# PFLeget/treegp

Hardware: AMD Instinct MI355X
Metric: GP solve+predict throughput, 2-D AnisotropicRBF N=65536 (higher is better)
Workload: dtype f64

## Files before the change

include/tgp.h:

```cpp
#ifndef TGP_H
#define TGP_H

#include <stdint.h>

#ifdef __cplusplus
extern "C" {
#endif

typedef struct tgp_ctx tgp_ctx;
typedef struct tgp_factor tgp_factor;

enum {
    TGP_RBF = 0,
    TGP_ARBF = 1,
    TGP_VK = 2,
    TGP_AVK = 3
};

typedef struct {
    int32_t kind;
    int32_t _pad;
    double amp;
    double a, b, c;
    double ell;
// ... 76 lines not shown
                 int k, double *out);

#define TGP_STAT_MEAN 0
#define TGP_STAT_MEDIAN 1
#define TGP_STAT_WEIGHTED 2
int tgp_binned_stat_2d(tgp_ctx *ctx, const double *u, const double *v, const double *val, const double *err,
                       int64_t n, const double *u_edges, int nu_edges, const double *v_edges, int nv_edges,
                       int stat, double *average, double *wrms, double *count);

int tgp_dev_alloc(tgp_ctx *ctx, int64_t bytes, void **d_out);
int tgp_dev_free(tgp_ctx *ctx, void *d_ptr);
int tgp_h2d(tgp_ctx *ctx, void *d_dst, const void *src, int64_t bytes);
int tgp_d2h(tgp_ctx *ctx, void *dst, const void *d_src, int64_t bytes);
int tgp_sync(tgp_ctx *ctx);
void *tgp_stream(tgp_ctx *ctx);
int tgp_mem_info(tgp_ctx *ctx, int64_t *free_bytes, int64_t *total_bytes);

int tgp_d_gp_solve(tgp_ctx *ctx, const tgp_kernel *k, const double *d_X, int64_t n,
                   const double *d_y, const double *d_yerr, double *d_alpha, double *logdet,
                   double *ydota, tgp_factor **keep);
int tgp_d_gp_predict(tgp_ctx *ctx, const tgp_kernel *k, const double *d_X, int64_t n,
                     const double *d_alpha, const double *d_Xs, int64_t m, double *d_ys);
int tgp_d_gp_solve_dense(tgp_ctx *ctx, const double *d_K, int64_t n, const double *d_y,
                         const double *d_yerr, double *d_alpha, double *logdet, double *ydota,
                         tgp_factor **keep);

int64_t tgp_panel_off(int64_t p, int64_t Np);
int64_t tgp_panel_elems(int64_t Np);
int64_t tgp_padded_n(int64_t n);

int tgp_d_kbuild_lower(tgp_ctx *ctx, const tgp_kernel *k, const double *d_X, int64_t n,
                       const double *d_yerr, double *d_A);
int tgp_d_potrf(tgp_ctx *ctx, double *d_A, int64_t Np, double *d_W);
int tgp_d_potrs(tgp_ctx *ctx, const double *d_A, const double *d_W, int64_t Np, double *d_b);
int tgp_d_potrs_multi(tgp_ctx *ctx, const double *d_A, const double *d_W, int64_t Np, double *d_B, int nrhs);
int tgp_d_unpack_lower(tgp_ctx *ctx, const double *d_A, int64_t Np, int64_t n, double *out);
int tgp_factor_device(tgp_ctx *ctx, const tgp_factor *f, const double **d_A, const double **d_W, int64_t *Np);
int tgp_set_stream(tgp_ctx *ctx, void *hip_stream);
int tgp_reset_stream(tgp_ctx *ctx);
int tgp_set_side_stream(tgp_ctx *ctx, void *hip_stream);
int64_t tgp_dist_panel_rows(int64_t p, int64_t Np, int G, int g);
int64_t tgp_dist_panel_off(int64_t p, int64_t Np, int G, int g);
int64_t tgp_dist_local_elems(int64_t Np, int G, int g);
int tgp_dd_kbuild(tgp_ctx *ctx, const tgp_kernel *k, const double *d_X, int64_t n, const double *d_yerr,
                  double *d_Aloc, const int64_t *d_loff, int G, int g);
int tgp_dd_factor_diag(tgp_ctx *ctx, double *d_Aloc, const int64_t *h_loff, int64_t Np, int kpanel, int G, int g,
                       double *d_W, double *d_bcast);
int tgp_dd_trsm(tgp_ctx *ctx, double *d_Aloc, const int64_t *h_loff, int64_t Np, int kpanel, int G, int g,
                double *d_W, const double *d_bcast);
int tgp_dd_update(tgp_ctx *ctx, double *d_Aloc, const int64_t *d_loff, int64_t Np, int kpanel, int G, int g,
                  const double *d_gathered, int cmax, int col_lo, int col_hi);
int tgp_dd_update2(tgp_ctx *ctx, double *d_Aloc, const int64_t *d_loff, int64_t Np, int kpanel, int G, int g,
                   const double *d_gathered0, int cmax0, const double *d_gathered1, int cmax1, int col_lo,
                   int col_hi);
int tgp_dd_update_group(tgp_ctx *ctx, double *d_Aloc, const int64_t *d_loff, int64_t Np, int kpanel, int G, int g,
                        int nseg, const double *const *d_gathered, const int *cmax, int col_lo, int col_hi);
int tgp_dd_strip_left(tgp_ctx *ctx, double *d_Aloc, const int64_t *h_loff, const int64_t *d_loff, int64_t Np, int kgroup, int b,
                      int G, int g, const double *d_ext);
int tgp_dd_queue_reset(tgp_ctx *ctx);
int tgp_dd_set_exclusive(tgp_ctx *ctx, int on);
int tgp_dd_update_group_queued(tgp_ctx *ctx, double *d_Aloc, const int64_t *d_loff, int64_t Np, int kpanel, int G, int g,
                               int nseg, const double *const *d_gathered, const int *cmax, int col_lo, int col_hi, int nres);
int tgp_dd_update_group_fused(tgp_ctx *ctx, double *d_Aloc, const int64_t *d_loff, int64_t Np, int kpanel, int G, int g, int nseg,
                              const double *const *d_gathered, const int *cmax, int head_cols, int nres);
int tgp_dd_wait_head(tgp_ctx *ctx, tgp_ctx *waiter);
int tgp_dd_tail_assemble(tgp_ctx *ctx, const double *d_gathered, int64_t stride, int64_t Np, int k0, int G, double *d_tail);
int tgp_dd_tail_scatter(tgp_ctx *ctx, const double *d_tail, int64_t Np, int k0, int G, int g, double *d_Aloc, const int64_t *d_loff);
int tgp_handoff_mode(tgp_ctx *ctx);
int tgp_dd_keep_panel(tgp_ctx *ctx, double *d_Afull, int64_t Np, int kpanel, int G, const double *d_bcast,
                      const double *d_gathered, int cmax);
int tgp_dd_fwd_diag(tgp_ctx *ctx, const double *d_Aloc, const int64_t *h_loff, int kb, const double *d_W, double *d_yk);
int tgp_dd_fwd_update(tgp_ctx *ctx, const double *d_Aloc, const int64_t *h_loff, int64_t Np, int kb, int G, int g,
                      const double *d_zk, double *d_yloc);
int tgp_dd_bwd_partial(tgp_ctx *ctx, const double *d_Aloc, const int64_t *h_loff, int64_t Np, int kb, int G, int g,
                       const double *d_aloc, double *d_s);
int tgp_dd_bwd_diag(tgp_ctx *ctx, const double *d_Aloc, const int64_t *h_loff, int kb, const double *d_W, double *d_ak,
                    const double *d_s );
int tgp_dd_logdet_local(tgp_ctx *ctx, const double *d_Aloc, const int64_t *d_loff, int64_t Np, int64_t n, int G, int g,
                        double *d_out);
int tgp_dd_info(tgp_ctx *ctx, int reset);

int tgp_debug_syrk_loop(tgp_ctx *ctx, double *d_A, int64_t Np, int reps, double *ms_per_launch,
                        double *flops_per_launch);
int tgp_debug_tilemap(int64_t T, int32_t *ti, int32_t *tj, int64_t cap);

#ifdef __cplusplus
}
#endif
#endif
```

treegp_amd/_lib.py:

```python
import ctypes as C
import os
import threading

import numpy as np

_HERE = os.path.dirname(os.path.abspath(__file__))
LIB_PATH = os.environ.get("TGP_LIB_PATH") or os.path.join(_HERE, "csrc", "libtgp.so")

TGP_RBF, TGP_ARBF, TGP_VK, TGP_AVK = 0, 1, 2, 3
NTIMINGS = 12


class TgpKernel(C.Structure):
    _fields_ = [("kind", C.c_int32), ("_pad", C.c_int32), ("amp", C.c_double), ("a", C.c_double),
                ("b", C.c_double), ("c", C.c_double), ("ell", C.c_double)]


_dp = C.POINTER(C.c_double)
_vp = C.c_void_p
_i64 = C.c_int64

SIGNATURES = {
    "tgp_init": (C.c_int, [C.POINTER(C.c_int), C.c_int, C.POINTER(_vp)]),
    "tgp_destroy": (None, [_vp]),
    "tgp_release_caches": (C.c_int, [_vp]),
    "tgp_last_error": (C.c_char_p, [_vp]),
    "tgp_version": (C.c_char_p, []),
    "tgp_device_count": (C.c_int, []),
    "tgp_last_timings": (C.c_int, [_vp, _dp, C.c_int]),
    "tgp_set_profiling": (C.c_int, [_vp, C.c_int]),
    "tgp_set_lookahead": (C.c_int, [_vp, C.c_int]),
    "tgp_kernel_matrix": (C.c_int, [_vp, C.POINTER(TgpKernel), _vp, _i64, _vp, _i64, _vp]),
    "tgp_gp_solve": (C.c_int, [_vp, C.POINTER(TgpKernel), _vp, _i64, _vp, _vp, _vp, _dp, _dp, C.POINTER(_vp)]),
    "tgp_factor_free": (None, [_vp, _vp]),
    "tgp_factor_release": (None, [_vp, _vp]),
    "tgp_factor_borrow": (C.c_int, [_vp, _vp, _vp, _i64, C.POINTER(_vp)]),
    "tgp_gp_predict": (C.c_int, [_vp, C.POINTER(TgpKernel), _vp, _i64, _vp, _vp, _i64, _vp]),
    "tgp_gp_predict_cov": (C.c_int, [_vp, _vp, C.POINTER(TgpKernel), _vp, _i64, _vp, _i64, _vp]),
    "tgp_kk_twod": (C.c_int, [_vp, _vp, _vp, _vp, _vp, _i64, C.c_double, C.c_double, C.c_int, _vp, _vp, _vp]),
    "tgp_kk_log": (C.c_int, [_vp, _vp, _vp, _vp, _vp, _i64, C.c_double, C.c_double, C.c_int, _vp, _vp, _vp, _vp, _vp]),
    "tgp_kk_partial": (C.c_int, [_vp, C.c_int, _vp, _vp, _vp, _vp, _i64, C.c_double, C.c_double, C.c_int, C.c_int, C.c_int, _vp]),
    "tgp_kk_twod_bootstrap": (C.c_int, [_vp, _vp, _vp, _vp, _vp, _i64, _vp, _i64, C.c_double, C.c_double, C.c_int, _vp]),
    "tgp_vcorr": (C.c_int, [_vp, _vp, _vp, _vp, _vp, _i64, _vp, C.c_int, _vp]),
    "tgp_knn_mean": (C.c_int, [_vp, _vp, _vp, _i64, _vp, _i64, C.c_int, _vp]),
    "tgp_binned_stat_2d": (C.c_int, [_vp, _vp, _vp, _vp, _vp, _i64, _vp, C.c_int, _vp, C.c_int, C.c_int, _vp, _vp, _vp]),
    "tgp_dev_alloc": (C.c_int, [_vp, _i64, C.POINTER(_vp)]),
    "tgp_dev_free": (C.c_int, [_vp, _vp]),
    "tgp_h2d": (C.c_int, [_vp, _vp, _vp, _i64]),
    "tgp_d2h": (C.c_int, [_vp, _vp, _vp, _i64]),
    "tgp_sync": (C.c_int, [_vp]),
    "tgp_stream": (_vp, [_vp]),
    "tgp_mem_info": (C.c_int, [_vp, C.POINTER(_i64), C.POINTER(_i64)]),
    "tgp_d_gp_solve": (C.c_int, [_vp, C.POINTER(TgpKernel), _vp, _i64, _vp, _vp, _vp, _dp, _dp, C.POINTER(_vp)]),
    "tgp_d_gp_predict": (C.c_int, [_vp, C.POINTER(TgpKernel), _vp, _i64, _vp, _vp, _i64, _vp]),
    "tgp_panel_off": (_i64, [_i64, _i64]),
    "tgp_panel_elems": (_i64, [_i64]),
    "tgp_padded_n": (_i64, [_i64]),
    "tgp_d_kbuild_lower": (C.c_int, [_vp, C.POINTER(TgpKernel), _vp, _i64, _vp, _vp]),
    "tgp_d_potrf": (C.c_int, [_vp, _vp, _i64, _vp]),
    "tgp_d_potrs": (C.c_int, [_vp, _vp, _vp, _i64, _vp]),
    "tgp_d_potrs_multi": (C.c_int, [_vp, _vp, _vp, _i64, _vp, C.c_int]),
    "tgp_gp_solve_dense": (C.c_int, [_vp, _vp, _i64, _vp, _vp, _vp, _dp, _dp, C.POINTER(_vp)]),
    "tgp_d_gp_solve_dense": (C.c_int, [_vp, _vp, _i64, _vp, _vp, _vp, _dp, _dp, C.POINTER(_vp)]),
    "tgp_factor_solve": (C.c_int, [_vp, _vp, _vp, C.c_int, _vp]),
    "tgp_factor_lmul": (C.c_int, [_vp, _vp, _vp, C.c_int, _vp]),
    "tgp_factor_inv_diag": (C.c_int, [_vp, _vp, _vp]),
    "tgp_gp_solve_batch": (C.c_int, [_vp, C.c_int, _vp, _vp, _i64, _vp, _vp, _vp, _vp, _vp, _vp, _vp]),
    "tgp_gp_posterior_batch": (C.c_int, [_vp, C.c_int, _vp, _vp, _i64, _vp, _vp, _vp, _vp, _i64, _vp, C.c_int, _vp, _vp, _vp, _vp, _vp]),
    "tgp_gp_predict_cov_dense": (C.c_int, [_vp, _vp, _vp, _vp, _i64, _vp]),
    "tgp_gp_predict_var": (C.c_int, [_vp, _vp, C.POINTER(TgpKernel), _vp, _i64, _vp, _i64, _vp]),
    "tgp_gp_predict_var_dense": (C.c_int, [_vp, _vp, _vp, _vp, _i64, _vp]),
    "tgp_gp_loglik_grad": (C.c_int, [_vp, _vp, C.POINTER(TgpKernel), _vp, _i64, _vp, _vp]),
    "tgp_d_gp_solve_grad": (C.c_int, [_vp, C.POINTER(TgpKernel), _vp, _i64, _vp, _vp, _dp, _dp, _vp]),
    "tgp_d_unpack_lower": (C.c_int, [_vp, _vp, _i64, _i64, _vp]),
    "tgp_factor_device": (C.c_int, [_vp, _vp, C.POINTER(_vp), C.POINTER(_vp), C.POINTER(_i64)]),
    "tgp_debug_syrk_loop": (C.c_int, [_vp, _vp, _i64, C.c_int, _dp, _dp]),
    "tgp_debug_tilemap": (C.c_int, [_i64, _vp, _vp, _i64]),
    "tgp_set_stream": (C.c_int, [_vp, _vp]),
    "tgp_reset_stream": (C.c_int, [_vp]),
    "tgp_set_side_stream": (C.c_int, [_vp, _vp]),
    "tgp_dist_panel_rows": (_i64, [_i64, _i64, C.c_int, C.c_int]),
    "tgp_dist_panel_off": (_i64, [_i64, _i64, C.c_int, C.c_int]),
    "tgp_dist_local_elems": (_i64, [_i64, C.c_int, C.c_int]),
    "tgp_dd_kbuild": (C.c_int, [_vp, C.POINTER(TgpKernel), _vp, _i64, _vp, _vp, _vp, C.c_int, C.c_int]),
    "tgp_dd_factor_diag": (C.c_int, [_vp, _vp, _vp, _i64, C.c_int, C.c_int, C.c_int, _vp, _vp]),
    "tgp_dd_trsm": (C.c_int, [_vp, _vp, _vp, _i64, C.c_int, C.c_int, C.c_int, _vp, _vp]),
    "tgp_dd_update": (C.c_int, [_vp, _vp, _vp, _i64, C.c_int, C.c_int, C.c_int, _vp, C.c_int, C.c_int, C.c_int]),
    "tgp_dd_update2": (C.c_int, [_vp, _vp, _vp, _i64, C.c_int, C.c_int, C.c_int, _vp, C.c_int, _vp, C.c_int, C.c_int, C.c_int]),
    "tgp_dd_update_group": (C.c_int, [_vp, _vp, _vp, _i64, C.c_int, C.c_int, C.c_int, C.c_int, _vp, _vp, C.c_int, C.c_int]),
    "tgp_dd_strip_left": (C.c_int, [_vp, _vp, _vp, _vp, _i64, C.c_int, C.c_int, C.c_int, C.c_int, _vp]),
    "tgp_dd_update_group_queued": (C.c_int, [_vp, _vp, _vp, _i64, C.c_int, C.c_int, C.c_int, C.c_int, _vp, _vp, C.c_int, C.c_int, C.c_int]),
    "tgp_dd_update_group_fused": (C.c_int, [_vp, _vp, _vp, _i64, C.c_int, C.c_int, C.c_int, C.c_int, _vp, _vp, C.c_int, C.c_int]),
    "tgp_dd_wait_head": (C.c_int, [_vp, _vp]),
    "tgp_handoff_mode": (C.c_int, [_vp]),
    "tgp_dd_tail_assemble": (C.c_int, [_vp, _vp, _i64, _i64, C.c_int, C.c_int, _vp]),
    "tgp_dd_tail_scatter": (C.c_int, [_vp, _vp, _i64, C.c_int, C.c_int, C.c_int, _vp, _vp]),
    "tgp_dd_queue_reset": (C.c_int, [_vp]),
    "tgp_dd_set_exclusive": (C.c_int, [_vp, C.c_int]),
    "tgp_dd_keep_panel": (C.c_int, [_vp, _vp, _i64, C.c_int, C.c_int, _vp, _vp, C.c_int]),
    "tgp_dd_fwd_diag": (C.c_int, [_vp, _vp, _vp, C.c_int, _vp, _vp]),
    "tgp_dd_fwd_update": (C.c_int, [_vp, _vp, _vp, _i64, C.c_int, C.c_int, C.c_int, _vp, _vp]),
    "tgp_dd_bwd_partial": (C.c_int, [_vp, _vp, _vp, _i64, C.c_int, C.c_int, C.c_int, _vp, _vp]),
    "tgp_dd_bwd_diag": (C.c_int, [_vp, _vp, _vp, C.c_int, _vp, _vp, _vp]),
    "tgp_dd_logdet_local": (C.c_int, [_vp, _vp, _vp, _i64, _i64, C.c_int, C.c_int, _vp]),
    "tgp_dd_info": (C.c_int, [_vp, C.c_int]),
}

_lib = None
_ctx = {}
_lock = threading.Lock()


def _share_hip_runtime_with_torch():
    import sys
    if "torch" in sys.modules or os.environ.get("TGP_SYSTEM_HIP") == "1":
        return
    try:
        import importlib.util
        spec = importlib.util.find_spec("torch")
        if spec is None or not spec.origin:
            return
        cand = os.path.join(os.path.dirname(spec.origin), "lib", "libamdhip64.so")
        if os.path.exists(cand):
            C.CDLL(cand, mode=C.RTLD_GLOBAL)
            if os.environ.get("TGP_VERBOSE"):
                print("treegp_amd: using torch's HIP runtime %s (one HIP runtime per process)" % cand, file=sys.stderr)
    except Exception:
        pass


def load_library():
    global _lib
    if _lib is None:
        if not os.path.exists(LIB_PATH):
            raise RuntimeError("libtgp.so not built (%s); run `python -c 'import __graft_entry__ as g; g.build()'` "
                               "or `make -C treegp_amd/csrc`" % LIB_PATH)
        _share_hip_runtime_with_torch()
        if os.environ.get("TGP_SET_HW_QUEUES", "1") != "0":
            os.environ.setdefault("GPU_MAX_HW_QUEUES", "8")
        lib = C.CDLL(LIB_PATH)
        for name, (res, args) in SIGNATURES.items():
            fn = getattr(lib, name)
            fn.restype = res
            fn.argtypes = args
        _lib = lib
    return _lib


class TgpError(RuntimeError):
    pass


_thread = threading.local()


def set_thread_ctx(ctx):
    _thread.ctx = ctx


def release_process_caches(device):
# ... 85 lines not shown
```

treegp_amd/csrc/chol.hip:

```cpp
#include "tgp_internal.h"

#include "gemm_tile.h"
#include "potrf128.h"

#ifdef TGP_POTRF_STAMPS
__device__ unsigned long long tgp_gemm_stamps[1024 * 4];
__device__ int tgp_gemm_stamp_grid = 43;
__device__ unsigned long long tgp_queue_stamps[1024 * 4];
__device__ int tgp_queue_stamp_T = 40;
__device__ unsigned long long tgp_mid_stamps[25 * 8];
__device__ int tgp_mid_stamp_base = 5120;
#define TGP_MID_STAMP(i)                                                                                   \
    do {                                                                                                   \
        if (threadIdx.x == 0 && base == tgp_mid_stamp_base && blockIdx.x < 25) tgp_mid_stamps[blockIdx.x * 8 + (i)] = __builtin_amdgcn_s_memrealtime(); \
    } while (0)
#else
#define TGP_MID_STAMP(i) ((void)0)
#endif

namespace {
template <int MODE, int LDB>
__global__ __launch_bounds__(256, 2) void gemm_col_kernel(const double *A, const double *B, double *C) {
    const int64_t t = blockIdx.x;
    TGP_CHAIN_PRIO();
// ... 504 lines not shown
            return hipFuncSetAttribute((const void *)panel_mid_kernel<true>, hipFuncAttributeMaxDynamicSharedMemorySize, (int)pad) == hipSuccess &&
                   hipFuncSetAttribute((const void *)panel_mid_kernel<false>, hipFuncAttributeMaxDynamicSharedMemorySize, (int)pad) == hipSuccess;
        }();
        const unsigned dyn = (exclusive && pad_ok) ? pad : 0u;
        if (17 + 8 * r2 <= cu_budget) panel_mid_kernel<true><<<25 + 8 * r2, 256, dyn, st>>>(Pk, W0, W1, d_info, base, mid_sync);
        else panel_mid_kernel<false><<<25 + r2, 256, dyn, st>>>(Pk, W0, W1, d_info, base, mid_sync);
    } else if (cu_budget > 0) {
        double *R2 = Pk + (int64_t)TGP_PW * TGP_PW;
        const bool small = 17 + 8 * r2 <= cu_budget;
        gemm_col_small_kernel<0, TGP_TB><<<8, 256, 0, st>>>(R1, W0, R1);
        if (r2 > 0) {
            if (small) gemm_col_small_kernel<0, TGP_TB><<<r2 * 8, 256, 0, st>>>(R2, W0, R2);
            else gemm_col_kernel<0, TGP_TB><<<r2, 256, 0, st>>>(R2, W0, R2);
        }
        gemm_col_small_kernel<1, TGP_PW><<<8, 256, 0, st>>>(R1, R1, R1 + TGP_TB);
        if (r2 > 0) {
            if (small) gemm_col_small_kernel<1, TGP_PW><<<r2 * 8, 256, 0, st>>>(R2, R1, R2 + TGP_TB);
            else gemm_col_kernel<1, TGP_PW><<<r2, 256, 0, st>>>(R2, R1, R2 + TGP_TB);
        }
        run_potrf128(st, R1 + TGP_TB, TGP_PW, W1, d_info, base + TGP_TB, exclusive, solo);
    } else {
        if (r1 <= small_rows) {
            gemm_col_small_kernel<0, TGP_TB><<<r1 * 8, 256, 0, st>>>(R1, W0, R1);
            gemm_col_small_kernel<1, TGP_PW><<<r1 * 8, 256, 0, st>>>(R1, R1, R1 + TGP_TB);
        } else {
            gemm_col_kernel<0, TGP_TB><<<r1, 256, 0, st>>>(R1, W0, R1);
            gemm_col_kernel<1, TGP_PW><<<r1, 256, 0, st>>>(R1, R1, R1 + TGP_TB);
        }
        run_potrf128(st, R1 + TGP_TB, TGP_PW, W1, d_info, base + TGP_TB, exclusive, solo);
    }
    if (r2 > 0) {
        double *R2 = Pk + (int64_t)TGP_PW * TGP_PW + TGP_TB;
        if (r2 <= small_rows) gemm_col_small_kernel<0, TGP_TB><<<r2 * 8, 256, 0, st>>>(R2, W1, R2);
        else gemm_col_kernel<0, TGP_TB><<<r2, 256, 0, st>>>(R2, W1, R2);
    }
}

inline int small_t() {
    static const int v = [] { const char *e = getenv("TGP_SMALL_T"); return e ? atoi(e) : 8; }();
    return v;
}

template <int NSEG>
void launch_syrk(hipStream_t st, double *d_A, int64_t Np, int ob, int T, int strip, const double *P0, const double *P1) {
    if (T <= 0) return;
    static const int strip_small_t = [] { const char *e = getenv("TGP_STRIP_SMALL_T"); return e ? atoi(e) : 16; }();
    if (T <= small_t() || (strip > 0 && T <= strip_small_t)) {
        const int cols = strip == 0 ? T : (strip < T ? strip : T);
        syrk_small_kernel<NSEG><<<dim3((unsigned)(T * 8), (unsigned)cols), 256, 0, st>>>(d_A, Np, ob, T, P0, P1);
        return;
    }
    static const int strip64_t = [] { const char *e = getenv("TGP_STRIP64_T"); return e ? atoi(e) : 128; }();
    static const int strip32_t = [] { const char *e = getenv("TGP_STRIP32_T"); return e ? atoi(e) : 64; }();
    if (strip > 0 && T <= strip32_t) {
        syrk_strip32_kernel<NSEG><<<(unsigned)((int64_t)4 * T * strip), 256, 0, st>>>(d_A, Np, ob, T, strip, P0, P1);
        return;
    }
    if (strip > 0 && T <= strip64_t) {
        syrk_strip64_kernel<NSEG><<<(unsigned)((int64_t)2 * T * strip), 256, 0, st>>>(d_A, Np, ob, T, strip, P0, P1);
        return;
    }
    const unsigned gs = strip == 0 ? (unsigned)tilemap_grid(T) : (unsigned)((int64_t)T * strip);
    syrk_dtv_kernel<NSEG><<<gs, 256, 0, st>>>(d_A, Np, ob, T, strip, P0, P1);
}

int queued_nres(int T) {
    static const int queue_res = [] { const char *e = getenv("TGP_QUEUE_RES"); return e ? atoi(e) : 0; }();
    if (queue_res > 0) return queue_res > TGP_QUEUE_MAXRES ? TGP_QUEUE_MAXRES : queue_res;
    static const int t1 = [] { const char *e = getenv("TGP_QUEUE_T1"); return e ? atoi(e) : 42; }();
    static const int t2 = [] { const char *e = getenv("TGP_QUEUE_T2"); return e ? atoi(e) : 26; }();
    return T >= t1 ? 1 : (T >= t2 ? 2 : 3);
}
void launch_syrk2_queued(tgp_ctx *ctx, hipStream_t st, double *d_A, int64_t Np, int ob, int T, const double *P0, const double *P1,
                         int nqueue) {
    const int nres = queued_nres(T);
    static const int half_env = [] { const char *e = getenv("TGP_QUEUE_HALF"); return e ? atoi(e) : -1; }();
    const unsigned slots = (unsigned)(tilemap_grid(T) / 8);
    unsigned nhalf = half_env >= 0 ? (unsigned)half_env : (unsigned)(512 - 64 * nres) / 8u;
    if (nhalf > slots) nhalf = slots;
    static const int steal = [] { const char *e = getenv("TGP_QUEUE_STEAL"); return e ? atoi(e) : 1; }();
    syrk_dtv_queue_kernel<2><<<512 + 8, 256, 0, st>>>(d_A, Np, ob, T, slots + nhalf, slots - nhalf, nres,
                                                     ctx->d_queue + TGP_QUEUE_WORDS * nqueue, P0, P1, steal);
}
}

int launch_potrf(tgp_ctx *ctx, double *d_A, int64_t Np, double *d_W, bool defer_info, int64_t n_data) {
    TGP_ARG(Np > 0 && Np % TGP_PW == 0);
    hipStream_t st = ctx->stream;
    TGP_HIP(hipMemsetAsync(ctx->d_info, 0, sizeof(int), st));
    const int nP = (int)(Np / TGP_PW);
    const bool prof = ctx->profiling != 0;
    if (prof) {
        while ((int)ctx->prof_events.size() < 2 * nP) {
            hipEvent_t e;
            TGP_HIP(hipEventCreate(&e));
            ctx->prof_events.push_back(e);
        }
    }
    static const int mode_env = [] { const char *e = getenv("TGP_CHOL_MODE"); return e ? atoi(e) : -1; }();
    const int mode = mode_env >= 0 ? mode_env : (!ctx->lookahead ? 1 : (Np >= 18432 ? 3 : (Np <= 1280 ? 1 : 2)));
    if (mode >= 2) {
        int rc = tgp_ensure_side_stream(ctx);
        if (rc) return rc;
    }
    double flops = 0.0;
    int nlaunch = 0;
    bool counting = true;
    auto timed = [&](auto &&fn, double fl) -> int {
        if (!counting) {
            fn();
            return 0;
        }
        if (prof) TGP_HIP(hipEventRecord(ctx->prof_events[2 * nlaunch], st));
        fn();
        if (prof) TGP_HIP(hipEventRecord(ctx->prof_events[2 * nlaunch + 1], st));
        flops += fl;
        ++nlaunch;
        return 0;
    };
    auto Wk = [&](int k) { return d_W + (int64_t)(2 * k) * TGP_TB * TGP_TB; };
    auto panel = [&](int k) { return d_A + panel_off(k, Np); };
    static const int queue_t = [] { const char *e = getenv("TGP_QUEUE_T"); return e ? atoi(e) : 64; }();
    int nqueue = 0;
    static const bool mid_env = [] { const char *e = getenv("TGP_PANEL_MID"); return e ? atoi(e) != 0 : true; }();
    const bool mid_on = mid_env && !ctx->mid_off && ctx->mid_allowed;
    if (mid_on) TGP_HIP(hipMemsetAsync(ctx->d_psync, 0, (size_t)(nP < TGP_PSYNC_PANELS ? nP : TGP_PSYNC_PANELS) * PANEL_SYNC_WORDS * sizeof(unsigned), st));
    if (Np / TGP_TB - 8 > small_t())
        TGP_HIP(hipMemsetAsync(ctx->d_queue, 0, TGP_NQUEUE * TGP_QUEUE_WORDS * sizeof(unsigned), st));
    auto psync = [&](int k) { return (mid_on && k < TGP_PSYNC_PANELS) ? ctx->d_psync + PANEL_SYNC_WORDS * k : nullptr; };
    auto run_pairs = [&](int kstart) -> int {
        hipStream_t sd = ctx->side_stream;
        auto factor_pair = [&](hipStream_t s, int k, bool exclusive = false, int cus = 0, bool tell = false) {
            const int64_t mk = Np - (int64_t)TGP_PW * k;
            auto sync = [&](int kk) { return (cus > 0 && mid_on && kk < TGP_PSYNC_PANELS) ? ctx->d_psync + PANEL_SYNC_WORDS * kk : nullptr; };
            factor_panel(s, panel(k), mk, Wk(k), ctx->d_info, k * TGP_PW, exclusive, n_data, sync(k), cus);
            if (tell) (void)tgp_signal(ctx, s, 2, ctx->ev[6]);
            if (k + 1 >= nP) return;
            const int T1 = (int)((mk - TGP_PW) / TGP_TB);
            launch_syrk<1>(s, d_A, Np, k + 1, T1, 2, panel(k) + (int64_t)TGP_PW * TGP_PW, nullptr);
            factor_panel(s, panel(k + 1), mk - TGP_PW, Wk(k + 1), ctx->d_info, (k + 1) * TGP_PW, exclusive, n_data, sync(k + 1), cus);
        };
        factor_pair(st, kstart, false, 256);
        static const int split_t = [] { const char *e = getenv("TGP_U2A_SPLIT_T"); return e ? atoi(e) : 64; }();
        bool early = false;
        for (int k = kstart; k + 2 < nP; k += 2) {
            const int T2 = (int)((Np - (int64_t)TGP_PW * (k + 2)) / TGP_TB);
            const double *P0 = panel(k) + (int64_t)2 * TGP_PW * TGP_PW;
            const double *P1 = panel(k + 1) + (int64_t)TGP_PW * TGP_PW;
            const int T3 = T2 - 4;
            const bool queued = T3 <= queue_t && T3 > small_t() && nqueue < TGP_NQUEUE;
            {
                const double rows = (double)T2 * TGP_TB, w = (T2 < 4 ? T2 : 4) * (double)TGP_TB;
                const double elems = w * (rows - w) + w * (w + 1.0) / 2.0;
                int rc = timed([&] {
                    if (early) launch_syrk<1>(st, d_A, Np, k + 2, T2, 4, P1, nullptr);
                    else launch_syrk<2>(st, d_A, Np, k + 2, T2, 4, P0, P1);
                }, (early ? 1.0 : 2.0) * 2.0 * TGP_PW * elems);
                if (rc) return rc;
            }
            TGP_HIP(tgp_signal(ctx, st, 0, ctx->ev[4]));
            TGP_HIP(tgp_await(ctx, sd, 0, ctx->ev[4]));
            const bool early_next = T3 > 0 && T3 <= split_t;
            factor_pair(sd, k + 2, queued, queued ? 32 * queued_nres(T3) : (T3 <= small_t() ? 256 : 0), early_next);
            TGP_HIP(tgp_signal(ctx, sd, 1, ctx->ev[5]));
            if (T3 > 0) {
                const double m = (double)T3 * TGP_TB;
                const int64_t skip = (int64_t)4 * TGP_TB * TGP_PW;
                int rc = timed([&] {
                    if (queued) launch_syrk2_queued(ctx, st, d_A, Np, k + 4, T3, P0 + skip, P1 + skip, nqueue++);
                    else launch_syrk<2>(st, d_A, Np, k + 4, T3, 0, P0 + skip, P1 + skip);
                }, 2.0 * TGP_PW * m * (m + 1.0));
                if (rc) return rc;
            }
            if (early_next) {
                TGP_HIP(tgp_await(ctx, st, 2, ctx->ev[6]));
                launch_syrk<1>(st, d_A, Np, k + 4, T3, 4, panel(k + 2) + (int64_t)2 * TGP_PW * TGP_PW, nullptr);
            }
            early = early_next;
            TGP_HIP(tgp_await(ctx, st, 1, ctx->ev[5]));
        }
        return 0;
    };
    if (mode == 0) {
        for (int k = 0; k < nP; ++k) {
            const int64_t mk = Np - (int64_t)TGP_PW * k;
            factor_panel(st, panel(k), mk, Wk(k), ctx->d_info, k * TGP_PW, false, n_data, psync(k), 256);
            const int T = (int)((mk - TGP_PW) / TGP_TB);
            if (T > 0) {
                const double m = (double)T * TGP_TB;
                int rc = timed([&] { launch_syrk<1>(st, d_A, Np, k + 1, T, 0, panel(k) + (int64_t)TGP_PW * TGP_PW, nullptr); },
                               (double)TGP_PW * m * (m + 1.0));
                if (rc) return rc;
            }
        }
    } else if (mode == 3) {
        hipStream_t sd = ctx->side_stream;
        auto seg_rows = [&](int kpanel, int first_block) {
            return (const double *)(panel(kpanel) + (int64_t)(first_block - kpanel) * TGP_PW * TGP_PW);
        };
        auto strip_update = [&](hipStream_t s, int k0, int j) {
            const int ob = k0 + j;
            const int T = (int)((Np - (int64_t)TGP_PW * ob) / TGP_TB);
            if (T <= small_t()) {
                for (int i = 0; i < j; ++i)
                    syrk_small_kernel<1><<<dim3((unsigned)(T * 8), 2u), 256, 0, s>>>(d_A, Np, ob, T, seg_rows(k0 + i, ob), nullptr);
                return;
            }
            const unsigned gs = (unsigned)((int64_t)T * 2);
            if (j == 1) {
                SegPtrs<1> P{{seg_rows(k0, ob)}, {nullptr}};
                syrk_segs_kernel<1><<<gs, 256, 0, s>>>(d_A, Np, ob, T, 2, P);
            } else if (j == 2) {
                SegPtrs<2> P{{seg_rows(k0, ob), seg_rows(k0 + 1, ob)}, {nullptr, nullptr}};
                syrk_segs_kernel<2><<<gs, 256, 0, s>>>(d_A, Np, ob, T, 2, P);
            } else {
                SegPtrs<3> P{{seg_rows(k0, ob), seg_rows(k0 + 1, ob), seg_rows(k0 + 2, ob)}, {nullptr, nullptr, nullptr}};
                syrk_segs_kernel<3><<<gs, 256, 0, s>>>(d_A, Np, ob, T, 2, P);
            }
        };
        auto factor_group = [&](hipStream_t s, int k0) {
            for (int j = 0; j < 4 && k0 + j < nP; ++j) {
                if (j > 0) strip_update(s, k0, j);
                factor_panel(s, panel(k0 + j), Np - (int64_t)TGP_PW * (k0 + j), Wk(k0 + j), ctx->d_info, (k0 + j) * TGP_PW, false, n_data);
            }
        };
        auto bulk = [&](int k0, int ob, int T, int strip) {
            if (T <= small_t()) {
                const int cols = strip == 0 ? T : (strip < T ? strip : T);
                for (int i = 0; i < 4; i += 2)
                    syrk_small_kernel<2><<<dim3((unsigned)(T * 8), (unsigned)cols), 256, 0, st>>>(
                        d_A, Np, ob, T, seg_rows(k0 + i, ob), seg_rows(k0 + i + 1, ob));
                return;
            }
            SegPtrs<4> P{{seg_rows(k0, ob), seg_rows(k0 + 1, ob), seg_rows(k0 + 2, ob), seg_rows(k0 + 3, ob)},
                         {nullptr, nullptr, nullptr, nullptr}};
            const unsigned gs = strip == 0 ? (unsigned)tilemap_grid(T) : (unsigned)((int64_t)T * strip);
            syrk_segs_kernel<4><<<gs, 256, 0, st>>>(d_A, Np, ob, T, strip, P);
        };
        static const int tail_tiles = [] { const char *e = getenv("TGP_QUAD_TAIL_TILES"); return e ? atoi(e) : 96; }();
        factor_group(st, 0);
        for (int k = 0; k + 4 < nP; k += 4) {
            const int T4 = (int)((Np - (int64_t)TGP_PW * (k + 4)) / TGP_TB);
            if (T4 <= tail_tiles) {
                const double m = (double)T4 * TGP_TB;
                int rc = timed([&] { bulk(k, k + 4, T4, 0); }, 4.0 * TGP_PW * m * (m + 1.0));
                if (rc) return rc;
                counting = false;
                rc = run_pairs(k + 4);
                counting = true;
                if (rc) return rc;
                break;
            }
            {
                const double rows = (double)T4 * TGP_TB, w = (T4 < 8 ? T4 : 8) * (double)TGP_TB;
                const double elems = w * (rows - w) + w * (w + 1.0) / 2.0;
                int rc = timed([&] { bulk(k, k + 4, T4, 8); }, 2.0 * 4.0 * TGP_PW * elems);
                if (rc) return rc;
            }
            TGP_HIP(tgp_signal(ctx, st, 0, ctx->ev[4]));
            TGP_HIP(tgp_await(ctx, sd, 0, ctx->ev[4]));
            factor_group(sd, k + 4);
            TGP_HIP(tgp_signal(ctx, sd, 1, ctx->ev[5]));
            const int T5 = T4 - 8;
            if (T5 > 0) {
                const double m = (double)T5 * TGP_TB;
                int rc = timed([&] { bulk(k, k + 8, T5, 0); }, 4.0 * TGP_PW * m * (m + 1.0));
                if (rc) return rc;
            }
            TGP_HIP(tgp_await(ctx, st, 1, ctx->ev[5]));
        }
    } else if (mode == 2) {
        int rc = run_pairs(0);
        if (rc) return rc;
    } else {
        for (int k = 0; k < nP; k += 2) {
            const int64_t mk = Np - (int64_t)TGP_PW * k;
            factor_panel(st, panel(k), mk, Wk(k), ctx->d_info, k * TGP_PW, false, n_data, psync(k), 256);
            if (k + 1 >= nP) break;
            const int T1 = (int)((mk - TGP_PW) / TGP_TB);
            launch_syrk<1>(st, d_A, Np, k + 1, T1, 2, panel(k) + (int64_t)TGP_PW * TGP_PW, nullptr);
            factor_panel(st, panel(k + 1), mk - TGP_PW, Wk(k + 1), ctx->d_info, (k + 1) * TGP_PW, false, n_data, psync(k + 1), 256);
            const int T2 = T1 - 2;
            if (T2 > 0) {
                const double m = (double)T2 * TGP_TB;
                int rc = timed([&] { launch_syrk<2>(st, d_A, Np, k + 2, T2, 0, panel(k) + (int64_t)2 * TGP_PW * TGP_PW,
                                                     panel(k + 1) + (int64_t)TGP_PW * TGP_PW); },
                               2.0 * TGP_PW * m * (m + 1.0));
                if (rc) return rc;
            }
        }
    }
    TGP_HIP(hipGetLastError());
    TGP_HIP(hipMemcpyAsync(ctx->h_info, ctx->d_info, sizeof(int), hipMemcpyDeviceToHost, st));
    ctx->timings[6] = nlaunch;
    ctx->timings[7] = flops;
    ctx->timings[5] = 0.0;
    if (defer_info && !prof) return 0;
    TGP_HIP(hipStreamSynchronize(st));
    if (prof) {
        double tot = 0.0;
        for (int i = 0; i < nlaunch; ++i) {
            float ms = 0.f;
            TGP_HIP(hipEventElapsedTime(&ms, ctx->prof_events[2 * i], ctx->prof_events[2 * i + 1]));
            tot += ms;
        }
        ctx->timings[5] = tot;
    }
    return tgp_potrf_info_rc(ctx, *ctx->h_info);
}

int tgp_potrf_info_rc(tgp_ctx *ctx, int info) {
    if (info >= 0) return info;
    ctx->err = "Cholesky: an in-kernel hand-off timed out (panel_mid_kernel waited 50 ms for workgroups of its own launch); "
               "the factor is incomplete -- TGP_PANEL_MID=0 selects the schedule without in-kernel waits";
    return TGP_RC_HANDOFF;
}

int launch_factor_diag256(tgp_ctx *ctx, double *blk, double *W0, double *W1, int base, bool latency) {
    hipStream_t st = ctx->stream;
    double *R1 = blk + (int64_t)TGP_TB * TGP_PW;
    const bool excl = ctx->chain_exclusive != 0;
    run_potrf128(st, blk, TGP_PW, W0, ctx->d_info, base, excl);
    if (latency) {
        gemm_col_small_kernel<0, TGP_TB><<<8, 256, 0, st>>>(R1, W0, R1);
        gemm_col_small_kernel<1, TGP_PW><<<8, 256, 0, st>>>(R1, R1, R1 + TGP_TB);
    } else {
        diag_mid_kernel<<<1, 256, 0, st>>>(R1, W0);
    }
    run_potrf128(st, R1 + TGP_TB, TGP_PW, W1, ctx->d_info, base + TGP_TB, excl);
    TGP_HIP(hipGetLastError());
    return 0;
}

int launch_trsm_rows(tgp_ctx *ctx, double *rows, int ntiles, const double *Lkk, const double *W0, const double *W1, double *keepW) {
    if (ntiles <= 0) {
        if (keepW) TGP_HIP(hipMemcpyAsync(keepW, W0, (size_t)2 * TGP_TB * TGP_TB * 8, hipMemcpyDeviceToDevice, ctx->stream));
        return 0;
    }
    constexpr int small_max = 24;
    if (ntiles <= small_max)
        panel_tall_small_kernel<<<ntiles * 8, 256, 0, ctx->stream>>>(rows, W0, Lkk + (int64_t)TGP_TB * TGP_PW, W1, keepW);
    else
        panel_tall_kernel<<<ntiles, 256, 0, ctx->stream>>>(rows, W0, Lkk + (int64_t)TGP_TB * TGP_PW, W1, keepW);
    TGP_HIP(hipGetLastError());
    return 0;
}

template <int NSEG>
static void launch_distn(hipStream_t st, unsigned grid, double *d_Aloc, const int64_t *d_loff, int kpanel, int G, int g,
                         const double *const *P, const int *cmax, int col_lo, int ncol, int nrows, const DistMap &M, int nres,
                         unsigned *queue, const double *const *PB) {
    DistSegs<NSEG> S;
    for (int s = 0; s < NSEG; ++s) {
        S.P[s] = P[s];
        S.PB[s] = PB ? PB[s] : P[s];
        S.cmax[s] = cmax[s];
        S.frg[s] = (int)dist_first_round(kpanel + s + 1, g, G);
    }
    if (nres > 0 && queue)
        syrk_distn_queue_kernel<NSEG><<<512 + 8, 256, 0, st>>>(d_Aloc, d_loff, kpanel, G, g, S, col_lo, ncol, nrows, M, grid / 8, nres, queue);
    else
        syrk_distn_kernel<NSEG><<<grid, 256, 0, st>>>(d_Aloc, d_loff, kpanel, G, g, S, col_lo, ncol, nrows, M);
}

int launch_syrk_distn(tgp_ctx *ctx, double *d_Aloc, const int64_t *d_loff, int64_t Np, int kpanel, int G, int g, int nseg,
                      const double *const *d_P, const int *cmax, int col_lo, int col_hi, int queue_nres, int head_cols,
                      const double *const *d_PB) {
    TGP_ARG(nseg >= 1 && nseg <= 4 && head_cols >= 0);
    const int64_t nB = Np / TGP_PW;
    const int64_t nloc = dist_panel_blocks(kpanel + nseg, nB, g, G);
    const int64_t ncol_all = 2 * (nB - kpanel - nseg);
    if (col_hi < 0 || col_hi > ncol_all) col_hi = (int)ncol_all;
    if (col_lo < 0) col_lo = 0;
    const int64_t ncol = (int64_t)col_hi - col_lo;
    hipStream_t st = ctx->stream;
    DistMap M;
    M.nhead = M.head_cols = M.whole = M.head_half = 0;
    M.half_from = 1 << 30;
    constexpr int half_max = 256;
    if (head_cols > 0) {
        hipError_t e = hipSuccess;
        M.hs.seq = tgp_next_seq(ctx, TGP_FLAG_HEAD, &e);
        TGP_HIP(e);
        M.hs.flag = ctx->d_flags + 16 * TGP_FLAG_HEAD;
        M.hs.done = ctx->d_flags + 16 * TGP_FLAG_HEAD_COUNT;
    }
    if (nloc <= 0 || ncol <= 0) {
        if (head_cols > 0) TGP_HIP(tgp_signal_value(ctx, st, TGP_FLAG_HEAD, M.hs.seq));
        return 0;
    }
    const int nrows = (int)(2 * nloc);
    const int64_t s0 = kpanel + nseg, qfb = dist_first_round(s0, g, G);
    M.qfb = (int)qfb;
    M.ginv = G == 1 ? 0u : (unsigned)((((uint64_t)1) << 32) / (uint64_t)G) + 1u;
    TGP_ARG(nB < 65536 && G >= 1);
    unsigned grid = 0;
    if (head_cols == 0 && ncol <= 8 && queue_nres == 0) {
        M.ngroups = 0;
        M.start[0] = 0;
        M.head_half = (int64_t)nrows * ncol <= half_max ? 1 : 0;
        grid = (unsigned)((int64_t)nrows * ncol) << M.head_half;
    } else {
        if (head_cols > ncol) head_cols = (int)ncol;
        M.head_cols = head_cols;
        M.head_half = (head_cols > 0 && (int64_t)nrows * head_cols <= half_max) ? 1 : 0;
        M.nhead = ((nrows * head_cols << M.head_half) + 7) / 8 * 8;
        M.ngroups = (nrows + 7) / 8;
        TGP_ARG(M.ngroups <= 257);
        int total = 0;
        for (int R = 0; R < M.ngroups; ++R) {
            M.start[R] = total;
            const int ltmax = (R * 8 + 7 < nrows ? R * 8 + 7 : nrows - 1);
            const int64_t gti = 2 * (dist_block_of(qfb + (ltmax >> 1), g, G) - s0) + (ltmax & 1);
            int64_t reach = gti - (col_lo + head_cols) + 1;
            if (reach > ncol - head_cols) reach = ncol - head_cols;
            total += reach > 0 ? (int)((reach + 7) / 8) : 0;
        }
        M.start[M.ngroups] = total;
        M.whole = 64 * (total / 8);
        const int slots = M.whole + 8 * (total % 8);
        static const int half_tiles = [] { const char *e = getenv("TGP_DIST_HALF_TILES"); return e ? atoi(e) : 32; }();
        const int nhalf = slots < half_tiles ? slots : half_tiles;
        M.half_from = slots - nhalf;
        grid = (unsigned)(M.nhead + 8 * (slots + nhalf));
        if (grid == 0) return 0;
        if (head_cols > 0) {
            ctx->head_count += (unsigned)M.nhead;
            M.hs.target = ctx->head_count;
        }
    }
    int nres = queue_nres > TGP_QUEUE_MAXRES ? TGP_QUEUE_MAXRES : queue_nres;
    unsigned *queue = nullptr;
    if (nres > 0 && M.ngroups != 0) {
        queue = ctx->d_queue + TGP_QUEUE_WORDS * (ctx->dist_nqueue % TGP_NQUEUE);
        if (ctx->dist_nqueue >= TGP_NQUEUE) TGP_HIP(hipMemsetAsync(queue, 0, TGP_QUEUE_WORDS * sizeof(unsigned), st));
        ++ctx->dist_nqueue;
    }
    switch (nseg) {
        case 1: launch_distn<1>(st, grid, d_Aloc, d_loff, kpanel, G, g, d_P, cmax, col_lo, (int)ncol, nrows, M, nres, queue, d_PB); break;
        case 2: launch_distn<2>(st, grid, d_Aloc, d_loff, kpanel, G, g, d_P, cmax, col_lo, (int)ncol, nrows, M, nres, queue, d_PB); break;
        case 3: launch_distn<3>(st, grid, d_Aloc, d_loff, kpanel, G, g, d_P, cmax, col_lo, (int)ncol, nrows, M, nres, queue, d_PB); break;
        default: launch_distn<4>(st, grid, d_Aloc, d_loff, kpanel, G, g, d_P, cmax, col_lo, (int)ncol, nrows, M, nres, queue, d_PB); break;
    }
    TGP_HIP(hipGetLastError());
    return 0;
}

int tgp_debug_syrk_loop(tgp_ctx *ctx, double *d_A, int64_t Np, int reps, double *ms_per_launch, double *flops_per_launch) {
    TGP_ARG(d_A && Np >= 4 * TGP_PW && Np % TGP_PW == 0 && reps > 0 && ms_per_launch && flops_per_launch);
    TGP_HIP(hipSetDevice(ctx->device));
    hipStream_t st = ctx->stream;
    const int T2 = (int)((Np - (int64_t)TGP_PW * 2) / TGP_TB);
    const double *P0 = d_A + panel_off(0, Np) + (int64_t)2 * TGP_PW * TGP_PW;
    const double *P1 = d_A + panel_off(1, Np) + (int64_t)TGP_PW * TGP_PW;
    if (getenv("TGP_DEBUG_SEGS")) {
        SegPtrs<4> P{{P0, P1, P0, P1}, {nullptr, nullptr, nullptr, nullptr}};
        const unsigned gs = (unsigned)tilemap_grid(T2);
        syrk_segs_kernel<4><<<gs, 256, 0, st>>>(d_A, Np, 2, T2, 0, P);
        TGP_HIP(hipEventRecord(ctx->ev[0], st));
        for (int r = 0; r < reps; ++r) syrk_segs_kernel<4><<<gs, 256, 0, st>>>(d_A, Np, 2, T2, 0, P);
        TGP_HIP(hipEventRecord(ctx->ev[1], st));
        TGP_HIP(hipStreamSynchronize(st));
        float ms2 = 0.f;
        TGP_HIP(hipEventElapsedTime(&ms2, ctx->ev[0], ctx->ev[1]));
        const double m2 = (double)T2 * TGP_TB;
        *ms_per_launch = ms2 / reps;
        *flops_per_launch = 4.0 * TGP_PW * m2 * (m2 + 1.0);
        return 0;
    }
    launch_syrk<2>(st, d_A, Np, 2, T2, 0, P0, P1);
    TGP_HIP(hipEventRecord(ctx->ev[0], st));
    for (int r = 0; r < reps; ++r) launch_syrk<2>(st, d_A, Np, 2, T2, 0, P0, P1);
    TGP_HIP(hipEventRecord(ctx->ev[1], st));
    TGP_HIP(hipStreamSynchronize(st));
    float ms = 0.f;
    TGP_HIP(hipEventElapsedTime(&ms, ctx->ev[0], ctx->ev[1]));
    const double m = (double)T2 * TGP_TB;
    *ms_per_launch = ms / reps;
    *flops_per_launch = 2.0 * TGP_PW * m * (m + 1.0);
    return 0;
}

#ifdef TGP_POTRF_STAMPS
extern "C" int tgp_debug_gemm_stamps(unsigned long long *out, int grid) {
    if (grid > 0) return (int)hipMemcpyToSymbol(HIP_SYMBOL(tgp_gemm_stamp_grid), &grid, sizeof(int));
    return (int)hipMemcpyFromSymbol(out, HIP_SYMBOL(tgp_gemm_stamps), 1024 * 4 * sizeof(unsigned long long));
}
extern "C" int tgp_debug_queue_stamps(unsigned long long *out, int T) {
    if (T > 0) return (int)hipMemcpyToSymbol(HIP_SYMBOL(tgp_queue_stamp_T), &T, sizeof(int));
    return (int)hipMemcpyFromSymbol(out, HIP_SYMBOL(tgp_queue_stamps), 1024 * 4 * sizeof(unsigned long long));
}
extern "C" int tgp_debug_mid_stamps(unsigned long long *out, int base) {
    if (base >= 0) return (int)hipMemcpyToSymbol(HIP_SYMBOL(tgp_mid_stamp_base), &base, sizeof(int));
    return (int)hipMemcpyFromSymbol(out, HIP_SYMBOL(tgp_mid_stamps), 25 * 8 * sizeof(unsigned long long));
}
extern "C" int tgp_debug_potrf_fine(unsigned long long *out) {
    return (int)hipMemcpyFromSymbol(out, HIP_SYMBOL(tgp_potrf_fine), 1024 * 8 * sizeof(unsigned long long));
}
extern "C" int tgp_debug_potrf_stamps(unsigned long long *out) {
    return (int)hipMemcpyFromSymbol(out, HIP_SYMBOL(tgp_potrf_stamps), 1024 * 20 * sizeof(unsigned long long));
}
#endif

int tgp_debug_tilemap(int64_t T, int32_t *ti, int32_t *tj, int64_t cap) {
    const int64_t g = tilemap_grid(T);
    if (cap < g) return -1;
    for (int64_t b = 0; b < g; ++b) {
        int i, j;
        tilemap(b, T, i, j);
        ti[b] = i;
        tj[b] = j;
    }
    return (int)g;
}
```

Baseline: 234,000.

## Plan Cholesky four-panel groups with a two-group lookahead window and 8-segment bulk SYRK

Measured after the change: 236,100 (median of 6 runs). About the same (+0.9%).

```diff
diff --git a/include/tgp.h b/include/tgp.h
--- a/include/tgp.h
+++ b/include/tgp.h
@@ -182,6 +182,11 @@
 
 int tgp_debug_syrk_loop(tgp_ctx *ctx, double *d_A, int64_t Np, int reps, double *ms_per_launch,
                         double *flops_per_launch);
+enum { TGP_PLAN_PANEL = 0, TGP_PLAN_STRIP = 1, TGP_PLAN_BULK = 2, TGP_PLAN_SIGNAL = 3, TGP_PLAN_AWAIT = 4, TGP_PLAN_PAIRS = 5 };
+typedef struct tgp_plan_launch {
+    int32_t stream, kind, p0, np, ob, T, strip, grid;
+} tgp_plan_launch;
+int tgp_debug_potrf_plan(int64_t Np, int window, int tail_tiles, int window_tiles, tgp_plan_launch *out, int64_t cap);
 int tgp_debug_tilemap(int64_t T, int32_t *ti, int32_t *tj, int64_t cap);
 
 #ifdef __cplusplus
diff --git a/treegp_amd/_lib.py b/treegp_amd/_lib.py
--- a/treegp_amd/_lib.py
+++ b/treegp_amd/_lib.py
@@ -76,6 +76,7 @@
     "tgp_factor_device": (C.c_int, [_vp, _vp, C.POINTER(_vp), C.POINTER(_vp), C.POINTER(_i64)]),
     "tgp_debug_syrk_loop": (C.c_int, [_vp, _vp, _i64, C.c_int, _dp, _dp]),
     "tgp_debug_tilemap": (C.c_int, [_i64, _vp, _vp, _i64]),
+    "tgp_debug_potrf_plan": (C.c_int, [_i64, C.c_int, C.c_int, C.c_int, _vp, _i64]),
     "tgp_set_stream": (C.c_int, [_vp, _vp]),
     "tgp_reset_stream": (C.c_int, [_vp]),
     "tgp_set_side_stream": (C.c_int, [_vp, _vp]),
diff --git a/treegp_amd/csrc/chol.hip b/treegp_amd/csrc/chol.hip
--- a/treegp_amd/csrc/chol.hip
+++ b/treegp_amd/csrc/chol.hip
@@ -610,6 +610,78 @@
     syrk_dtv_queue_kernel<2><<<512 + 8, 256, 0, st>>>(d_A, Np, ob, T, slots + nhalf, slots - nhalf, nres,
                                                      ctx->d_queue + TGP_QUEUE_WORDS * nqueue, P0, P1, steal);
 }
+
+void potrf_plan_fours(std::vector<tgp_plan_launch> &out, int64_t Np, int W, int tail_tiles, int win_tiles, int small_rows_t) {
+    const int nP = (int)(Np / TGP_PW);
+    auto tiles_from = [&](int blk) { return blk >= nP ? 0 : (int)((Np - (int64_t)TGP_PW * blk) / TGP_TB); };
+    auto push = [&](int stream, int kind, int p0, int np, int ob, int T, int strip, int64_t grid) {
+        out.push_back(tgp_plan_launch{stream, kind, p0, np, ob, T, strip, (int32_t)grid});
+    };
+    int G = 1;
+    for (int k = 0; k + 4 < nP && tiles_from(k + 4) > tail_tiles; k += 4) ++G;
+    auto group = [&](int stream, int g) {
+        const int k0 = 4 * g;
+        for (int j = 0; j < 4 && k0 + j < nP; ++j) {
+            const int T = tiles_from(k0 + j);
+            if (j > 0) push(stream, TGP_PLAN_STRIP, k0, j, k0 + j, T, 2, T <= small_rows_t ? (int64_t)T * 8 * 2 * j : (int64_t)T * 2);
+            push(stream, TGP_PLAN_PANEL, k0 + j, 1, k0 + j, T, 0, 0);
+        }
+    };
+    auto bulk = [&](int stream, int p0, int np, int ob, int strip) {
+        const int T = tiles_from(ob);
+        if (T <= 0 || np <= 0) return;
+        const int cols = strip == 0 ? T : (strip < T ? strip : T);
+        const int64_t grid = T <= small_rows_t ? (int64_t)T * 8 * cols * ((np + 1) / 2) : (strip == 0 ? tilemap_grid(T) : (int64_t)T * strip);
+        push(stream, TGP_PLAN_BULK, p0, np, ob, T, strip, grid);
+    };
+    auto choose = [&](int next) {
+        const int left = G - next;
+        if (left <= 0) return 0;
+        const int Tn = tiles_from(4 * next);
+        return (W > 1 && Tn > win_tiles && Tn - 8 * W - 8 > small_rows_t) ? (W < left ? W : left) : 1;
+    };
+    int first = 0, pend = choose(0);
+    for (int g = 0; g < pend; ++g) {
+        if (g > 0) bulk(0, 0, 4 * g, 4 * g, 8);
+        group(0, g);
+    }
+    for (;;) {
+        const int next = first + pend, p0 = 4 * first;
+        const int np = 4 * pend < nP - p0 ? 4 * pend : nP - p0;
+        const int r = choose(next);
+        if (r == 0) {
+            if (4 * next < nP) {
+                bulk(0, p0, np, 4 * next, 0);
+                push(0, TGP_PLAN_PAIRS, 4 * next, nP - 4 * next, 4 * next, tiles_from(4 * next), 0, 0);
+            }
+            break;
+        }
+        bulk(0, p0, np, 4 * next, 8 * r);
+        push(0, TGP_PLAN_SIGNAL, 0, 0, 0, 0, 0, 0);
+        push(1, TGP_PLAN_AWAIT, 0, 0, 0, 0, 0, 0);
+        for (int g = 0; g < r; ++g) {
+            if (g > 0) bulk(1, 4 * next, 4 * g, 4 * (next + g), 8);
+            group(1, next + g);
+        }
+        push(1, TGP_PLAN_SIGNAL, 1, 0, 0, 0, 0, 0);
+        bulk(0, p0, np, 4 * (next + r), 0);
+        push(0, TGP_PLAN_AWAIT, 1, 0, 0, 0, 0, 0);
+        first = next;
+        pend = r;
+    }
+}
+int quad_tail_tiles() {
+    static const int v = [] { const char *e = getenv("TGP_QUAD_TAIL_TILES"); return e ? atoi(e) : 96; }();
+    return v;
+}
+int bulk_window() {
+    static const int v = [] { const char *e = getenv("TGP_BULK_WINDOW"); const int w = e ? atoi(e) : 2; return w < 1 ? 1 : (w > 2 ? 2 : w); }();
+    return v;
+}
+int bulk_window_tiles() {
+    static const int v = [] { const char *e = getenv("TGP_BULK_WINDOW_TILES"); return e ? atoi(e) : 256; }();
+    return v;
+}
 }
 
 int launch_potrf(tgp_ctx *ctx, double *d_A, int64_t Np, double *d_W, bool defer_info, int64_t n_data) {
@@ -634,14 +706,17 @@
     double flops = 0.0;
     int nlaunch = 0;
     bool counting = true;
-    auto timed = [&](auto &&fn, double fl) -> int {
+    int nclocked = 0;
+    auto timed = [&](hipStream_t ts, auto &&fn, double fl, bool clocked = true) -> int {
         if (!counting) {
             fn();
             return 0;
         }
-        if (prof) TGP_HIP(hipEventRecord(ctx->prof_events[2 * nlaunch], st));
+        const bool ev = prof && clocked;
+        if (ev) TGP_HIP(hipEventRecord(ctx->prof_events[2 * nclocked], ts));
         fn();
-        if (prof) TGP_HIP(hipEventRecord(ctx->prof_events[2 * nlaunch + 1], st));
+        if (ev) TGP_HIP(hipEventRecord(ctx->prof_events[2 * nclocked + 1], ts));
+        if (ev) ++nclocked;
         flops += fl;
         ++nlaunch;
         return 0;
@@ -680,7 +755,7 @@
             {
                 const double rows = (double)T2 * TGP_TB, w = (T2 < 4 ? T2 : 4) * (double)TGP_TB;
                 const double elems = w * (rows - w) + w * (w + 1.0) / 2.0;
-                int rc = timed([&] {
+                int rc = timed(st, [&] {
                     if (early) launch_syrk<1>(st, d_A, Np, k + 2, T2, 4, P1, nullptr);
                     else launch_syrk<2>(st, d_A, Np, k + 2, T2, 4, P0, P1);
                 }, (early ? 1.0 : 2.0) * 2.0 * TGP_PW * elems);
@@ -694,7 +769,7 @@
             if (T3 > 0) {
                 const double m = (double)T3 * TGP_TB;
                 const int64_t skip = (int64_t)4 * TGP_TB * TGP_PW;
-                int rc = timed([&] {
+                int rc = timed(st, [&] {
                     if (queued) launch_syrk2_queued(ctx, st, d_A, Np, k + 4, T3, P0 + skip, P1 + skip, nqueue++);
                     else launch_syrk<2>(st, d_A, Np, k + 4, T3, 0, P0 + skip, P1 + skip);
                 }, 2.0 * TGP_PW * m * (m + 1.0));
@@ -716,7 +791,7 @@
             const int T = (int)((mk - TGP_PW) / TGP_TB);
             if (T > 0) {
                 const double m = (double)T * TGP_TB;
-                int rc = timed([&] { launch_syrk<1>(st, d_A, Np, k + 1, T, 0, panel(k) + (int64_t)TGP_PW * TGP_PW, nullptr); },
+                int rc = timed(st, [&] { launch_syrk<1>(st, d_A, Np, k + 1, T, 0, panel(k) + (int64_t)TGP_PW * TGP_PW, nullptr); },
                                (double)TGP_PW * m * (m + 1.0));
                 if (rc) return rc;
             }
@@ -746,56 +821,57 @@
                 syrk_segs_kernel<3><<<gs, 256, 0, s>>>(d_A, Np, ob, T, 2, P);
             }
         };
-        auto factor_group = [&](hipStream_t s, int k0) {
-            for (int j = 0; j < 4 && k0 + j < nP; ++j) {
-                if (j > 0) strip_update(s, k0, j);
-                factor_panel(s, panel(k0 + j), Np - (int64_t)TGP_PW * (k0 + j), Wk(k0 + j), ctx->d_info, (k0 + j) * TGP_PW, false, n_data);
-            }
-        };
-        auto bulk = [&](int k0, int ob, int T, int strip) {
+        auto bulk = [&](hipStream_t s, int k0, int np, int ob, int T, int strip) {
             if (T <= small_t()) {
                 const int cols = strip == 0 ? T : (strip < T ? strip : T);
-                for (int i = 0; i < 4; i += 2)
-                    syrk_small_kernel<2><<<dim3((unsigned)(T * 8), (unsigned)cols), 256, 0, st>>>(
+                for (int i = 0; i < np; i += 2)
+                    syrk_small_kernel<2><<<dim3((unsigned)(T * 8), (unsigned)cols), 256, 0, s>>>(
                         d_A, Np, ob, T, seg_rows(k0 + i, ob), seg_rows(k0 + i + 1, ob));
                 return;
             }
-            SegPtrs<4> P{{seg_rows(k0, ob), seg_rows(k0 + 1, ob), seg_rows(k0 + 2, ob), seg_rows(k0 + 3, ob)},
-                         {nullptr, nullptr, nullptr, nullptr}};
             const unsigned gs = strip == 0 ? (unsigned)tilemap_grid(T) : (unsigned)((int64_t)T * strip);
-            syrk_segs_kernel<4><<<gs, 256, 0, st>>>(d_A, Np, ob, T, strip, P);
+            if (np == 4) {
+                SegPtrs<4> P{{seg_rows(k0, ob), seg_rows(k0 + 1, ob), seg_rows(k0 + 2, ob), seg_rows(k0 + 3, ob)},
+                             {nullptr, nullptr, nullptr, nullptr}};
+                syrk_segs_kernel<4><<<gs, 256, 0, s>>>(d_A, Np, ob, T, strip, P);
+            } else {
+                SegPtrs<8> P{};
+                for (int i = 0; i < 8; ++i) P.a[i] = seg_rows(k0 + i, ob);
+                syrk_segs_kernel<8><<<gs, 256, 0, s>>>(d_A, Np, ob, T, strip, P);
+            }
         };
-        static const int tail_tiles = [] { const char *e = getenv("TGP_QUAD_TAIL_TILES"); return e ? atoi(e) : 96; }();
-        factor_group(st, 0);
-        for (int k = 0; k + 4 < nP; k += 4) {
-            const int T4 = (int)((Np - (int64_t)TGP_PW * (k + 4)) / TGP_TB);
-            if (T4 <= tail_tiles) {
-                const double m = (double)T4 * TGP_TB;
-                int rc = timed([&] { bulk(k, k + 4, T4, 0); }, 4.0 * TGP_PW * m * (m + 1.0));
+        std::vector<tgp_plan_launch> plan;
+        potrf_plan_fours(plan, Np, bulk_window(), quad_tail_tiles(), bulk_window_tiles(), small_t());
+        for (const tgp_plan_launch &L : plan) {
+            hipStream_t s = L.stream ? sd : st;
+            switch (L.kind) {
+            case TGP_PLAN_PANEL:
+                factor_panel(s, panel(L.p0), Np - (int64_t)TGP_PW * L.p0, Wk(L.p0), ctx->d_info, L.p0 * TGP_PW, false, n_data);
+                break;
+            case TGP_PLAN_STRIP: strip_update(s, L.p0, L.np); break;
+            case TGP_PLAN_BULK: {
+                TGP_ARG(L.np == 4 || L.np == 8);
+                double elems;
+                if (L.strip == 0) {
+                    const double m = (double)L.T * TGP_TB;
+                    elems = m * (m + 1.0) / 2.0;
+                } else {
+                    const double rows = (double)L.T * TGP_TB, w = (L.T < L.strip ? L.T : L.strip) * (double)TGP_TB;
+                    elems = w * (rows - w) + w * (w + 1.0) / 2.0;
+                }
+                int rc = timed(s, [&] { bulk(s, L.p0, L.np, L.ob, L.T, L.strip); }, 2.0 * L.np * TGP_PW * elems, L.stream == 0);
                 if (rc) return rc;
+                break;
+            }
+            case TGP_PLAN_SIGNAL: TGP_HIP(tgp_signal(ctx, s, L.p0, ctx->ev[4 + L.p0])); break;
+            case TGP_PLAN_AWAIT: TGP_HIP(tgp_await(ctx, s, L.p0, ctx->ev[4 + L.p0])); break;
+            default: {
                 counting = false;
-                rc = run_pairs(k + 4);
+                int rc = run_pairs(L.p0);
                 counting = true;
                 if (rc) return rc;
-                break;
-            }
-            {
-                const double rows = (double)T4 * TGP_TB, w = (T4 < 8 ? T4 : 8) * (double)TGP_TB;
-                const double elems = w * (rows - w) + w * (w + 1.0) / 2.0;
-                int rc = timed([&] { bulk(k, k + 4, T4, 8); }, 2.0 * 4.0 * TGP_PW * elems);
-                if (rc) return rc;
-            }
-            TGP_HIP(tgp_signal(ctx, st, 0, ctx->ev[4]));
-            TGP_HIP(tgp_await(ctx, sd, 0, ctx->ev[4]));
-            factor_group(sd, k + 4);
-            TGP_HIP(tgp_signal(ctx, sd, 1, ctx->ev[5]));
-            const int T5 = T4 - 8;
-            if (T5 > 0) {
-                const double m = (double)T5 * TGP_TB;
-                int rc = timed([&] { bulk(k, k + 8, T5, 0); }, 4.0 * TGP_PW * m * (m + 1.0));
-                if (rc) return rc;
-            }
-            TGP_HIP(tgp_await(ctx, st, 1, ctx->ev[5]));
+            }
+            }
         }
     } else if (mode == 2) {
         int rc = run_pairs(0);
@@ -811,7 +887,7 @@
             const int T2 = T1 - 2;
             if (T2 > 0) {
                 const double m = (double)T2 * TGP_TB;
-                int rc = timed([&] { launch_syrk<2>(st, d_A, Np, k + 2, T2, 0, panel(k) + (int64_t)2 * TGP_PW * TGP_PW,
+                int rc = timed(st, [&] { launch_syrk<2>(st, d_A, Np, k + 2, T2, 0, panel(k) + (int64_t)2 * TGP_PW * TGP_PW,
                                                      panel(k + 1) + (int64_t)TGP_PW * TGP_PW); },
                                2.0 * TGP_PW * m * (m + 1.0));
                 if (rc) return rc;
@@ -827,7 +903,7 @@
     TGP_HIP(hipStreamSynchronize(st));
     if (prof) {
         double tot = 0.0;
-        for (int i = 0; i < nlaunch; ++i) {
+        for (int i = 0; i < nclocked; ++i) {
             float ms = 0.f;
             TGP_HIP(hipEventElapsedTime(&ms, ctx->prof_events[2 * i], ctx->prof_events[2 * i + 1]));
             tot += ms;
@@ -981,19 +1057,25 @@
     const int T2 = (int)((Np - (int64_t)TGP_PW * 2) / TGP_TB);
     const double *P0 = d_A + panel_off(0, Np) + (int64_t)2 * TGP_PW * TGP_PW;
     const double *P1 = d_A + panel_off(1, Np) + (int64_t)TGP_PW * TGP_PW;
-    if (getenv("TGP_DEBUG_SEGS")) {
+    if (const char *segs = getenv("TGP_DEBUG_SEGS")) {
+        const bool deep = atoi(segs) == 8;
         SegPtrs<4> P{{P0, P1, P0, P1}, {nullptr, nullptr, nullptr, nullptr}};
+        SegPtrs<8> Q{{P0, P1, P0, P1, P0, P1, P0, P1}, {}};
         const unsigned gs = (unsigned)tilemap_grid(T2);
-        syrk_segs_kernel<4><<<gs, 256, 0, st>>>(d_A, Np, 2, T2, 0, P);
+        auto launch = [&] {
+            if (deep) syrk_segs_kernel<8><<<gs, 256, 0, st>>>(d_A, Np, 2, T2, 0, Q);
+            else syrk_segs_kernel<4><<<gs, 256, 0, st>>>(d_A, Np, 2, T2, 0, P);
+        };
+        launch();
         TGP_HIP(hipEventRecord(ctx->ev[0], st));
-        for (int r = 0; r < reps; ++r) syrk_segs_kernel<4><<<gs, 256, 0, st>>>(d_A, Np, 2, T2, 0, P);
+        for (int r = 0; r < reps; ++r) launch();
         TGP_HIP(hipEventRecord(ctx->ev[1], st));
         TGP_HIP(hipStreamSynchronize(st));
         float ms2 = 0.f;
         TGP_HIP(hipEventElapsedTime(&ms2, ctx->ev[0], ctx->ev[1]));
         const double m2 = (double)T2 * TGP_TB;
         *ms_per_launch = ms2 / reps;
-        *flops_per_launch = 4.0 * TGP_PW * m2 * (m2 + 1.0);
+        *flops_per_launch = (deep ? 8.0 : 4.0) * TGP_PW * m2 * (m2 + 1.0);
         return 0;
     }
     launch_syrk<2>(st, d_A, Np, 2, T2, 0, P0, P1);
@@ -1030,6 +1112,16 @@
 }
 #endif
 
+int tgp_debug_potrf_plan(int64_t Np, int window, int tail_tiles, int window_tiles, tgp_plan_launch *out, int64_t cap) {
+    if (Np <= 0 || Np % TGP_PW != 0 || (cap > 0 && !out)) return -2;
+    std::vector<tgp_plan_launch> plan;
+    potrf_plan_fours(plan, Np, window > 0 ? window : bulk_window(), tail_tiles >= 0 ? tail_tiles : quad_tail_tiles(),
+                     window_tiles >= 0 ? window_tiles : bulk_window_tiles(), small_t());
+    if ((int64_t)plan.size() > cap) return -1;
+    for (size_t i = 0; i < plan.size(); ++i) out[i] = plan[i];
+    return (int)plan.size();
+}
+
 int tgp_debug_tilemap(int64_t T, int32_t *ti, int32_t *tj, int64_t cap) {
     const int64_t g = tilemap_grid(T);
     if (cap < g) return -1;
```
